# Eclectic-Sheep/sheeprl

Measured on NVIDIA H100. Metric: Dreamer-V3 train-steps/sec (S, bs16 seq64 horizon15, 64x64x3 obs), higher is better.
Workload: dtype f32

## Files before the change

sheeprl_b200/csrc/gemm_tc.cu:

```cuda
#include <cuda.h>
#include <cudaTypedefs.h>

#include <mutex>
#include <unordered_map>

#include "common.cuh"

namespace {

constexpr int BM = 128, BK = 32;
constexpr int NTHREADS = 384;
constexpr int NSPLIT_THREADS = 96;
constexpr int NCONS_WARPS = 8;
constexpr int PRODUCER_REGS = 56, CONSUMER_REGS = 224;
template <int PASSES, bool PRESPLIT> __host__ __device__ constexpr int b_buffers() { return PRESPLIT ? (PASSES == 3 ? 2 : 1) : 3; }
template <int BN, int PASSES, bool PRESPLIT> constexpr int stages_for() {
  return (227 * 1024 - 1024 - 256) / ((BM + b_buffers<PASSES, PRESPLIT>() * BN) * BK * (int)sizeof(float));
}

__device__ __forceinline__ uint32_t smem_u32(const void* p) { return (uint32_t)__cvta_generic_to_shared(p); }

__device__ __forceinline__ void mbar_init(uint64_t* bar, uint32_t count) {
  asm volatile("mbarrier.init.shared::cta.b64 [%0], %1;" ::"r"(smem_u32(bar)), "r"(count) : "memory");
}
__device__ __forceinline__ void mbar_expect_tx(uint64_t* bar, uint32_t bytes) {
  asm volatile("mbarrier.arrive.expect_tx.shared::cta.b64 _, [%0], %1;" ::"r"(smem_u32(bar)), "r"(bytes) : "memory");
}
__device__ __forceinline__ void mbar_arrive(uint64_t* bar) {
  asm volatile("mbarrier.arrive.shared::cta.b64 _, [%0];" ::"r"(smem_u32(bar)) : "memory");
}
__device__ __forceinline__ bool mbar_try_wait(uint64_t* bar, uint32_t parity) {
  uint32_t ok;
  asm volatile(
      "{\n\t"
      ".reg .pred p;\n\t"
      "mbarrier.try_wait.parity.shared::cta.b64 p, [%1], %2;\n\t"
      "selp.u32 %0, 1, 0, p;\n\t"
      "}"
      : "=r"(ok)
      : "r"(smem_u32(bar)), "r"(parity)
      : "memory");
  return ok != 0;
}
__device__ __forceinline__ void mbar_wait(uint64_t* bar, uint32_t parity) {
  if (mbar_try_wait(bar, parity)) return;
  const long long t0 = clock64();
  while (!mbar_try_wait(bar, parity)) {
    if (clock64() - t0 > 2000000000LL) asm volatile("trap;");
  }
}
__device__ __forceinline__ bool elect_one() {
  uint32_t pred;
  asm volatile(
      "{\n\t"
      ".reg .pred p;\n\t"
      "elect.sync _|p, 0xffffffff;\n\t"
      "selp.u32 %0, 1, 0, p;\n\t"
      "}"
      : "=r"(pred));
  return pred != 0;
}
__device__ __forceinline__ void tma_load_2d(void* smem_dst, const CUtensorMap* map, uint64_t* bar, int c0, int c1) {
  asm volatile(
      "cp.async.bulk.tensor.2d.shared::cluster.global.mbarrier::complete_tx::bytes [%0], [%1, {%3, %4}], [%2];" ::"r"(
          smem_u32(smem_dst)),
      "l"(map), "r"(smem_u32(bar)), "r"(c0), "r"(c1)
      : "memory");
}
__device__ __forceinline__ void tma_load_4d(void* smem_dst, const CUtensorMap* map, uint64_t* bar, int c0, int c1, int c2,
                                            int c3) {
  asm volatile(
      "cp.async.bulk.tensor.4d.shared::cluster.global.mbarrier::complete_tx::bytes [%0], [%1, {%3, %4, %5, %6}], [%2];" ::"r"(
          smem_u32(smem_dst)),
      "l"(map), "r"(smem_u32(bar)), "r"(c0), "r"(c1), "r"(c2), "r"(c3)
      : "memory");
}

__device__ __forceinline__ void wgmma_tf32(float (&d)[32], const uint32_t (&a)[4], uint64_t desc_b, int scale_d) {
  asm volatile(
      "{\n\t.reg .pred p;\n\tsetp.ne.b32 p, %37, 0;\n\twgmma.mma_async.sync.aligned.m64n64k8.f32.tf32.tf32 {%0, %1, %2, %3, %4, %5, %6, %7, %8, %9, %10, %11, %12, %13, %14, %15, %16, %17, %18, %19, %20, %21, %22, %23, %24, %25, %26, %27, %28, %29, %30, %31}, {%32, %33, %34, %35}, %36, p, 1, 1;\n\t}"
      : "+f"(d[0]), "+f"(d[1]), "+f"(d[2]), "+f"(d[3]), "+f"(d[4]), "+f"(d[5]), "+f"(d[6]), "+f"(d[7]), "+f"(d[8]), "+f"(d[9]), "+f"(d[10]), "+f"(d[11]), "+f"(d[12]), "+f"(d[13]), "+f"(d[14]), "+f"(d[15]), "+f"(d[16]), "+f"(d[17]), "+f"(d[18]), "+f"(d[19]), "+f"(d[20]), "+f"(d[21]), "+f"(d[22]), "+f"(d[23]), "+f"(d[24]), "+f"(d[25]), "+f"(d[26]), "+f"(d[27]), "+f"(d[28]), "+f"(d[29]), "+f"(d[30]), "+f"(d[31])
      : "r"(a[0]), "r"(a[1]), "r"(a[2]), "r"(a[3]), "l"(desc_b), "r"(scale_d));
}
__device__ __forceinline__ void wgmma_tf32(float (&d)[64], const uint32_t (&a)[4], uint64_t desc_b, int scale_d) {
  asm volatile(
      "{\n\t.reg .pred p;\n\tsetp.ne.b32 p, %69, 0;\n\twgmma.mma_async.sync.aligned.m64n128k8.f32.tf32.tf32 {%0, %1, %2, %3, %4, %5, %6, %7, %8, %9, %10, %11, %12, %13, %14, %15, %16, %17, %18, %19, %20, %21, %22, %23, %24, %25, %26, %27, %28, %29, %30, %31, %32, %33, %34, %35, %36, %37, %38, %39, %40, %41, %42, %43, %44, %45, %46, %47, %48, %49, %50, %51, %52, %53, %54, %55, %56, %57, %58, %59, %60, %61, %62, %63}, {%64, %65, %66, %67}, %68, p, 1, 1;\n\t}"
      : "+f"(d[0]), "+f"(d[1]), "+f"(d[2]), "+f"(d[3]), "+f"(d[4]), "+f"(d[5]), "+f"(d[6]), "+f"(d[7]), "+f"(d[8]), "+f"(d[9]), "+f"(d[10]), "+f"(d[11]), "+f"(d[12]), "+f"(d[13]), "+f"(d[14]), "+f"(d[15]), "+f"(d[16]), "+f"(d[17]), "+f"(d[18]), "+f"(d[19]), "+f"(d[20]), "+f"(d[21]), "+f"(d[22]), "+f"(d[23]), "+f"(d[24]), "+f"(d[25]), "+f"(d[26]), "+f"(d[27]), "+f"(d[28]), "+f"(d[29]), "+f"(d[30]), "+f"(d[31]), "+f"(d[32]), "+f"(d[33]), "+f"(d[34]), "+f"(d[35]), "+f"(d[36]), "+f"(d[37]), "+f"(d[38]), "+f"(d[39]), "+f"(d[40]), "+f"(d[41]), "+f"(d[42]), "+f"(d[43]), "+f"(d[44]), "+f"(d[45]), "+f"(d[46]), "+f"(d[47]), "+f"(d[48]), "+f"(d[49]), "+f"(d[50]), "+f"(d[51]), "+f"(d[52]), "+f"(d[53]), "+f"(d[54]), "+f"(d[55]), "+f"(d[56]), "+f"(d[57]), "+f"(d[58]), "+f"(d[59]), "+f"(d[60]), "+f"(d[61]), "+f"(d[62]), "+f"(d[63])
      : "r"(a[0]), "r"(a[1]), "r"(a[2]), "r"(a[3]), "l"(desc_b), "r"(scale_d));
}
__device__ __forceinline__ void wgmma_fence() { asm volatile("wgmma.fence.sync.aligned;" ::: "memory"); }
__device__ __forceinline__ void wgmma_commit() { asm volatile("wgmma.commit_group.sync.aligned;" ::: "memory"); }
__device__ __forceinline__ void wgmma_wait_all() { asm volatile("wgmma.wait_group.sync.aligned 0;" ::: "memory"); }
template <int N>
__device__ __forceinline__ void fence_regs(float (&r)[N]) {
#pragma unroll
  for (int i = 0; i < N; ++i) asm volatile("" : "+f"(r[i])::"memory");
}
template <int N, int W>
__device__ __forceinline__ void fence_regs(uint32_t (&r)[N][W]) {
#pragma unroll
  for (int i = 0; i < N; ++i)
#pragma unroll
    for (int j = 0; j < W; ++j) asm volatile("" : "+r"(r[i][j])::"memory");
}

__device__ __forceinline__ uint64_t make_desc(uint32_t smem_addr) {
  uint64_t d = 0;
  d |= (uint64_t)((smem_addr & 0x3FFFF) >> 4);
  d |= (uint64_t)1 << 16;
  d |= (uint64_t)(1024 >> 4) << 32;
  d |= (uint64_t)1 << 62;
  return d;
}

__device__ __forceinline__ uint32_t kmajor_off(int r, int k) {
  return (uint32_t)(r * 128 + ((((k >> 2) ^ r) & 7) << 4) + (k & 3) * 4);
}
__device__ __forceinline__ uint32_t mnmajor_off(int r, int k) {
  return (uint32_t)((r >> 5) * 4096 + k * 128 + (((((r & 31) >> 2) ^ k) & 7) << 4) + (r & 3) * 4);
}

template <int BN, int PASSES, bool PRESPLIT>
struct Smem;
template <int BN, int PASSES>
struct Smem<BN, PASSES, false> {
  static constexpr int STAGES = stages_for<BN, PASSES, false>();
  float a[STAGES][BM * BK];
  float b[STAGES][BN * BK];
  float b_hi[STAGES][BN * BK];
  float b_lo[STAGES][BN * BK];
  uint64_t full[STAGES], split[STAGES], empty[STAGES];
};
template <int BN, int PASSES>
struct Smem<BN, PASSES, true> {
  static constexpr int STAGES = stages_for<BN, PASSES, true>();
  float a[STAGES][BM * BK];
  float b_hi[STAGES][BN * BK];
  float b_lo[PASSES == 3 ? STAGES : 1][PASSES == 3 ? BN * BK : 256];
  uint64_t full[STAGES], empty[STAGES];
};

constexpr int CH = 4;

constexpr int MODE_GEMM = 0, MODE_DOWN = 1, MODE_UP = 2;
constexpr int MODE_UP4 = 3;
constexpr int GROUP_M = 16;
struct TileGeo {
  int mode;
  int h, w, NB;
  int bw, bh, bn;
  int tiles_x, tiles_y;
  int chunks;
  int Cout;
  int ksplits;
  float* part;
  int mpad, ldw;
  int force_part;
  int passes;
  int a_mn, b_mn;
  int mtiles;
  int ntiles;
  int wg;
};

template <int BN, int PASSES, bool PRESPLIT>
__global__ void __launch_bounds__(NTHREADS, 1)
gemm_tc_kernel(const __grid_constant__ CUtensorMap mapA, const __grid_constant__ CUtensorMap mapB,
               const __grid_constant__ CUtensorMap mapBlo, float* __restrict__ C, const float* __restrict__ bias, int M,
               int N, int K, int ldc, int accumulate, const TileGeo geo) {
  using S = Smem<BN, PASSES, PRESPLIT>;
  constexpr int STAGES = S::STAGES;
  extern __shared__ __align__(1024) unsigned char smem_raw[];
  S& s = *reinterpret_cast<S*>(smem_raw + ((1024u - (smem_u32(smem_raw) & 1023u)) & 1023u));
  const int warp = threadIdx.x >> 5, lane = threadIdx.x & 31;
  const int mtiles = geo.mtiles * geo.ntiles, tstride = gridDim.y;
  auto tile_mn = [&](int id, int& tm, int& tn) {
    if (geo.ntiles == 1) { tm = id; tn = 0; return; }
    const int per = GROUP_M * geo.ntiles, grp = id / per, first = grp * GROUP_M;
    const int gsz = min(GROUP_M, geo.mtiles - first), r = id - grp * per;
    tn = r / gsz;
    tm = first + (r - tn * gsz);
  };
  int kb_base = 0, nkb = (K + BK - 1) / BK;
  if (geo.mode == MODE_GEMM && geo.ksplits > 1) {
    const int per = (nkb + geo.ksplits - 1) / geo.ksplits;
    kb_base = (int)blockIdx.z * per;
    nkb = min(per, nkb - kb_base);
  }
  const int py = (int)blockIdx.z >> 1, px = (int)blockIdx.z & 1;
  auto tile_origin = [&](int id, int& tx0, int& ty0, int& tn0) {
    tx0 = (id % geo.tiles_x) * geo.bw;
    ty0 = ((id / geo.tiles_x) % geo.tiles_y) * geo.bh;
    tn0 = (id / (geo.tiles_x * geo.tiles_y)) * geo.bn;
  };

  if (threadIdx.x == 0) {
    for (int i = 0; i < STAGES; ++i) {
      mbar_init(&s.full[i], 1);
      if constexpr (!PRESPLIT) mbar_init(&s.split[i], NSPLIT_THREADS / 32);
      mbar_init(&s.empty[i], NCONS_WARPS);
    }
    asm volatile("fence.mbarrier_init.release.cluster;" ::: "memory");
  }
  __syncthreads();

  if (warp < 4) {
    asm volatile("setmaxnreg.dec.sync.aligned.u32 %0;" ::"n"(PRODUCER_REGS));
    if (warp == 0) {
      const bool leader = elect_one();
      constexpr uint32_t STAGE_TX = (uint32_t)((BM + (PRESPLIT ? b_buffers<PASSES, true>() : 1) * BN) * BK * sizeof(float));
      auto load_b_kmajor = [&](int st, int k, int n) {
        if constexpr (PRESPLIT) {
          tma_load_2d(s.b_hi[st], &mapB, &s.full[st], k, n);
          if (PASSES == 3) tma_load_2d(s.b_lo[st], &mapBlo, &s.full[st], k, n);
        } else {
          tma_load_2d(s.b[st], &mapB, &s.full[st], k, n);
        }
      };
      int it = 0;
      for (int tile = blockIdx.y; tile < mtiles; tile += tstride) {
        int tm, tn;
        tile_mn(tile, tm, tn);
        const int m0 = tm * BM, n0 = tn * BN;
        int tx0 = 0, ty0 = 0, tn0 = 0;
        if (geo.mode != MODE_GEMM) tile_origin(tm, tx0, ty0, tn0);
        for (int kb = 0; kb < nkb; ++kb, ++it) {
          const int st = it % STAGES;
          if (it >= STAGES) mbar_wait(&s.empty[st], ((it / STAGES) - 1) & 1);
          if (leader) {
            mbar_expect_tx(&s.full[st], STAGE_TX);
            if (geo.mode == MODE_GEMM) {
              const int k0 = (kb_base + kb) * BK;
              if (geo.wg) {
                const int x0 = k0 % geo.w, y0 = (k0 / geo.w) % geo.h, i0 = k0 / (geo.w * geo.h);
                for (int j = 0; j < BM / 32; ++j) {
                  const int r0 = m0 + 32 * j, tap = r0 / geo.Cout, ch = r0 - tap * geo.Cout;
                  tma_load_4d(s.a[st] + j * 1024, &mapA, &s.full[st], ch, 2 * x0 - 1 + (tap & 3), 2 * y0 - 1 + (tap >> 2), i0);
                }
              } else if (!geo.a_mn) tma_load_2d(s.a[st], &mapA, &s.full[st], k0, m0);
              else
                for (int j = 0; j < BM / 32; ++j) tma_load_2d(s.a[st] + j * 1024, &mapA, &s.full[st], m0 + 32 * j, k0);
              if (PRESPLIT || !geo.b_mn) load_b_kmajor(st, k0, n0);
              else if constexpr (!PRESPLIT)
                for (int j = 0; j < BN / 32; ++j) tma_load_2d(s.b[st] + j * 1024, &mapB, &s.full[st], n0 + 32 * j, k0);
            } else {
              const int tap = kb / geo.chunks, ch = (kb - tap * geo.chunks) * BK;
              int x, y;
              if (geo.mode == MODE_DOWN)     { x = 2 * tx0 - 1 + (tap & 3); y = 2 * ty0 - 1 + (tap >> 2); }
              else if (geo.mode == MODE_UP4) { x = tx0 + (tap % 3) - 1;     y = ty0 + (tap / 3) - 1; }
              else                           { x = tx0 + px - (tap & 1);    y = ty0 + py - (tap >> 1); }
              tma_load_4d(s.a[st], &mapA, &s.full[st], ch, x, y, tn0);
              load_b_kmajor(st, kb * BK, n0 + (geo.mode == MODE_UP ? (int)blockIdx.z * geo.Cout : 0));
            }
          }
          __syncwarp();
        }
      }
    } else if constexpr (!PRESPLIT) {
      const int t = threadIdx.x - 32;
      int ntl = 0;
      for (int tile = blockIdx.y; tile < mtiles; tile += tstride) ++ntl;
      const int total_kb = ntl * nkb;
      const bool b_mn = geo.b_mn != 0;
      for (int kb = 0; kb < total_kb; ++kb) {
        const int st = kb % STAGES;
        mbar_wait(&s.full[st], (kb / STAGES) & 1);
        const char* raw = reinterpret_cast<const char*>(s.b[st]);
        char* bh = reinterpret_cast<char*>(s.b_hi[st]);
        char* bl = reinterpret_cast<char*>(s.b_lo[st]);
#pragma unroll 4
        for (int w = t; w < BN * BK / 4; w += NSPLIT_THREADS) {
          int n, kc;
          float4 v;
          if (!b_mn) {
            n = w >> 3; kc = w & 7;
            v = *reinterpret_cast<const float4*>(raw + kmajor_off(n, 4 * kc));
          } else {
            n = w % BN; kc = w / BN;
            v.x = *reinterpret_cast<const float*>(raw + mnmajor_off(n, 4 * kc));
            v.y = *reinterpret_cast<const float*>(raw + mnmajor_off(n, 4 * kc + 1));
            v.z = *reinterpret_cast<const float*>(raw + mnmajor_off(n, 4 * kc + 2));
            v.w = *reinterpret_cast<const float*>(raw + mnmajor_off(n, 4 * kc + 3));
          }
          float4 h;
          h.x = __uint_as_float(__float_as_uint(v.x) & 0xffffe000u);
          h.y = __uint_as_float(__float_as_uint(v.y) & 0xffffe000u);
          h.z = __uint_as_float(__float_as_uint(v.z) & 0xffffe000u);
          h.w = __uint_as_float(__float_as_uint(v.w) & 0xffffe000u);
          const uint32_t o = kmajor_off(n, 4 * kc);
          *reinterpret_cast<float4*>(bh + o) = h;
          if (PASSES == 3) *reinterpret_cast<float4*>(bl + o) = make_float4(v.x - h.x, v.y - h.y, v.z - h.z, v.w - h.w);
        }
        asm volatile("fence.proxy.async.shared::cta;" ::: "memory");
        __syncwarp();
        if (lane == 0) mbar_arrive(&s.split[st]);
      }
    }
  } else {
    asm volatile("setmaxnreg.inc.sync.aligned.u32 %0;" ::"n"(CONSUMER_REGS));
    constexpr int NACC = BN / 2;
    const int cw = (warp >> 2) - 1, wq = warp & 3, g = lane >> 2, tq = lane & 3;
    const int r0 = cw * 64 + wq * 16 + g;
    const bool a_mn_tile = geo.a_mn != 0;
    const uint64_t dbh_base = make_desc(smem_u32(s.b_hi[0])), dbl_base = make_desc(smem_u32(s.b_lo[0]));
    constexpr uint64_t STAGE_STEP = (uint64_t)(BN * BK * sizeof(float)) >> 4;
    int it = 0;
    for (int tile = blockIdx.y; tile < mtiles; tile += tstride) {
      int tm, tn;
      tile_mn(tile, tm, tn);
      const int m0 = tm * BM, n0 = tn * BN;
      int tx0 = 0, ty0 = 0, tn0 = 0;
      if (geo.mode != MODE_GEMM) tile_origin(tm, tx0, ty0, tn0);
      float acc[NACC], cacc[NACC];
#pragma unroll
      for (int j = 0; j < NACC; ++j) { acc[j] = 0.f; cacc[j] = 0.f; }
      for (int kb = 0; kb < nkb; ++kb, ++it) {
        const int st = it % STAGES;
        const uint32_t ph = (it / STAGES) & 1;
        mbar_wait(&s.full[st], ph);
        if constexpr (!PRESPLIT) mbar_wait(&s.split[st], ph);
        const char* araw = reinterpret_cast<const char*>(s.a[st]);
        uint32_t ahi[4][4], alo[4][4];
#pragma unroll
        for (int ks = 0; ks < 4; ++ks)
#pragma unroll
          for (int e = 0; e < 4; ++e) {
            const int r = r0 + 8 * (e & 1), k = 8 * ks + tq + 4 * (e >> 1);
            const uint32_t x = *reinterpret_cast<const uint32_t*>(araw + (a_mn_tile ? mnmajor_off(r, k) : kmajor_off(r, k)));
            ahi[ks][e] = x & 0xffffe000u;
            if (PASSES == 3) alo[ks][e] = __float_as_uint(__uint_as_float(x) - __uint_as_float(x & 0xffffe000u));
          }
        const bool chunk_start = (kb % CH) == 0;
        const uint64_t dbh0 = dbh_base + (uint64_t)st * STAGE_STEP, dbl0 = dbl_base + (uint64_t)st * STAGE_STEP;
        fence_regs(cacc);
        fence_regs(ahi);
        if (PASSES == 3) fence_regs(alo);
        wgmma_fence();
#pragma unroll
        for (int ks = 0; ks < 4; ++ks) {
          const uint64_t ob = (uint64_t)ks * 2;
          const int keep = !(chunk_start && ks == 0);
          if (PASSES == 3) {
            wgmma_tf32(cacc, ahi[ks], dbl0 + ob, keep);
            wgmma_tf32(cacc, alo[ks], dbh0 + ob, 1);
            wgmma_tf32(cacc, ahi[ks], dbh0 + ob, 1);
          } else {
            wgmma_tf32(cacc, ahi[ks], dbh0 + ob, keep);
          }
        }
        wgmma_commit();
        wgmma_wait_all();
        fence_regs(cacc);
        fence_regs(ahi);
        if (PASSES == 3) fence_regs(alo);
        __syncwarp();
        if (lane == 0) mbar_arrive(&s.empty[st]);
        if ((kb % CH) == CH - 1 || kb == nkb - 1) {
#pragma unroll
          for (int j = 0; j < NACC; ++j) acc[j] += cacc[j];
        }
      }
#pragma unroll
      for (int hh = 0; hh < 2; ++hh) {
        const int r = r0 + 8 * hh;
        const int row = m0 + r;
        bool row_ok = row < M;
        size_t row_off = (size_t)row * ldc;
        int wi = 0, hi = 0, ni = 0;
        if (geo.mode != MODE_GEMM) {
          wi = r % geo.bw; hi = (r / geo.bw) % geo.bh; ni = r / (geo.bw * geo.bh);
          const int n = tn0 + ni, y = ty0 + hi, x = tx0 + wi;
          row_ok = n < geo.NB;
          if (geo.mode == MODE_DOWN) row_off = (((size_t)n * geo.h + y) * geo.w + x) * (size_t)ldc;
          else row_off = (((size_t)n * (2 * geo.h) + (2 * y + py)) * (2 * geo.w) + (2 * x + px)) * (size_t)ldc;
        }
        if (geo.mode == MODE_UP4) {
          if (!row_ok) continue;
          const size_t n = (size_t)(tn0 + ni);
          const int y = ty0 + hi, x = tx0 + wi;
#pragma unroll
          for (int j = 0; j < NACC / 4; ++j) {
            const int c = 8 * j + 2 * tq, p = c >> 5, ch = c & 31;
            float* dst = C + ((n * (2 * geo.h) + (2 * y + (p >> 1))) * (2 * geo.w) + (2 * x + (p & 1))) * (size_t)32 + ch;
            float2 o = make_float2(acc[4 * j + 2 * hh], acc[4 * j + 2 * hh + 1]);
            if (bias) { o.x += bias[ch]; o.y += bias[ch + 1]; }
            *reinterpret_cast<float2*>(dst) = o;
          }
          continue;
        }
        if (geo.mode == MODE_GEMM && (geo.ksplits > 1 || geo.force_part)) {
          float* prow = geo.part + ((size_t)blockIdx.z * geo.mpad + (size_t)row) * geo.ldw + n0;
#pragma unroll
          for (int j = 0; j < NACC / 4; ++j)
            *reinterpret_cast<float2*>(prow + 8 * j + 2 * tq) = make_float2(acc[4 * j + 2 * hh], acc[4 * j + 2 * hh + 1]);
          continue;
        }
        if (!row_ok) continue;
        float* crow = C + row_off;
#pragma unroll
        for (int j = 0; j < NACC / 4; ++j) {
          const int cb = n0 + 8 * j + 2 * tq;
          float v0 = acc[4 * j + 2 * hh], v1 = acc[4 * j + 2 * hh + 1];
          if (cb + 1 < N && ((reinterpret_cast<uintptr_t>(crow + cb) & 7) == 0)) {
            if (bias) { v0 += bias[cb]; v1 += bias[cb + 1]; }
            if (accumulate) { const float2 q = *reinterpret_cast<const float2*>(crow + cb); v0 += q.x; v1 += q.y; }
            *reinterpret_cast<float2*>(crow + cb) = make_float2(v0, v1);
          } else {
            if (cb < N) crow[cb] = v0 + (bias ? bias[cb] : 0.f) + (accumulate ? crow[cb] : 0.f);
            if (cb + 1 < N) crow[cb + 1] = v1 + (bias ? bias[cb + 1] : 0.f) + (accumulate ? crow[cb + 1] : 0.f);
          }
        }
      }
    }
  }
}

struct MapKey {
  const void* ptr; int rows, cols, ld, box_rows;
  bool operator==(const MapKey& o) const { return ptr == o.ptr && rows == o.rows && cols == o.cols && ld == o.ld && box_rows == o.box_rows; }
};
struct MapHash {
  size_t operator()(const MapKey& k) const {
    size_t h = std::hash<const void*>()(k.ptr);
    h ^= std::hash<long long>()(((long long)k.rows << 32) ^ k.cols) + 0x9e3779b97f4a7c15ull + (h << 6) + (h >> 2);
    h ^= std::hash<long long>()(((long long)k.ld << 8) ^ k.box_rows) + 0x9e3779b97f4a7c15ull + (h << 6) + (h >> 2);
    return h;
  }
};
std::unordered_map<MapKey, CUtensorMap, MapHash> g_maps;
std::mutex g_maps_mu;

typedef CUresult (*EncodeTiledFn)(CUtensorMap*, CUtensorMapDataType, cuuint32_t, void*, const cuuint64_t*, const cuuint64_t*,
                                  const cuuint32_t*, const cuuint32_t*, CUtensorMapInterleave, CUtensorMapSwizzle,
                                  CUtensorMapL2promotion, CUtensorMapFloatOOBfill);
EncodeTiledFn encode_tiled() {
  static EncodeTiledFn fn = nullptr;
  if (!fn) {
    void* p = nullptr;
    cudaDriverEntryPointQueryResult q;
    if (cudaGetDriverEntryPoint("cuTensorMapEncodeTiled", &p, cudaEnableDefault, &q) == cudaSuccess &&
        q == cudaDriverEntryPointSuccess)
      fn = reinterpret_cast<EncodeTiledFn>(p);
  }
  return fn;
}

int get_map(const float* ptr, int rows, int cols, int ld, int box_rows, CUtensorMap* out) {
  MapKey key{ptr, rows, cols, ld, box_rows};
  std::lock_guard<std::mutex> lk(g_maps_mu);
  auto it = g_maps.find(key);
  if (it != g_maps.end()) { *out = it->second; return B200RL_OK; }
  CUtensorMap m;
  cuuint64_t dims[2] = {(cuuint64_t)cols, (cuuint64_t)rows};
  cuuint64_t strides[1] = {(cuuint64_t)ld * sizeof(float)};
  cuuint32_t box[2] = {(cuuint32_t)BK, (cuuint32_t)box_rows};
  cuuint32_t estr[2] = {1, 1};
  EncodeTiledFn enc = encode_tiled();
  if (!enc) { b200rl_set_error("cuTensorMapEncodeTiled is not available from this driver"); return B200RL_ERR_CUDA; }
  CUresult r = enc(&m, CU_TENSOR_MAP_DATA_TYPE_FLOAT32, 2, const_cast<float*>(ptr), dims, strides, box,
                                      estr, CU_TENSOR_MAP_INTERLEAVE_NONE,
                                      CU_TENSOR_MAP_SWIZZLE_128B,
                                      CU_TENSOR_MAP_L2_PROMOTION_L2_256B, CU_TENSOR_MAP_FLOAT_OOB_FILL_NONE);
  if (r != CUDA_SUCCESS) {
    b200rl_set_error("cuTensorMapEncodeTiled failed (%d) for [%d x %d] ld %d", (int)r, rows, cols, ld);
    return B200RL_ERR_CUDA;
  }
  if (g_maps.size() > 4096) g_maps.clear();
  g_maps.emplace(key, m);
  *out = m;
  return B200RL_OK;
}

struct Map4Key {
  const void* ptr; int C, W, H, N, bw, bh, bn, es;
  bool operator==(const Map4Key& o) const {
    return ptr == o.ptr && C == o.C && W == o.W && H == o.H && N == o.N && bw == o.bw && bh == o.bh && bn == o.bn && es == o.es;
  }
};
struct Map4Hash {
  size_t operator()(const Map4Key& k) const {
    size_t h = std::hash<const void*>()(k.ptr);
    const long long v[4] = {((long long)k.C << 32) ^ k.W, ((long long)k.H << 32) ^ k.N, ((long long)k.bw << 32) ^ k.bh,
                            ((long long)k.bn << 32) ^ k.es};
    for (long long x : v) h ^= std::hash<long long>()(x) + 0x9e3779b97f4a7c15ull + (h << 6) + (h >> 2);
    return h;
  }
};
std::unordered_map<Map4Key, CUtensorMap, Map4Hash> g_maps4;

int get_map4(const float* ptr, int C, int W, int H, int N, int bw, int bh, int bn, int es, CUtensorMap* out) {
  Map4Key key{ptr, C, W, H, N, bw, bh, bn, es};
  std::lock_guard<std::mutex> lk(g_maps_mu);
  auto it = g_maps4.find(key);
  if (it != g_maps4.end()) { *out = it->second; return B200RL_OK; }
  CUtensorMap m;
  cuuint64_t dims[4] = {(cuuint64_t)C, (cuuint64_t)W, (cuuint64_t)H, (cuuint64_t)N};
  cuuint64_t strides[3] = {(cuuint64_t)C * 4, (cuuint64_t)C * W * 4, (cuuint64_t)C * W * H * 4};
  cuuint32_t box[4] = {(cuuint32_t)BK, (cuuint32_t)((bw - 1) * es + 1), (cuuint32_t)((bh - 1) * es + 1), (cuuint32_t)bn};
  cuuint32_t estr[4] = {1, (cuuint32_t)es, (cuuint32_t)es, 1};
  EncodeTiledFn enc = encode_tiled();
  if (!enc) { b200rl_set_error("cuTensorMapEncodeTiled is not available from this driver"); return B200RL_ERR_CUDA; }
  CUresult r = enc(&m, CU_TENSOR_MAP_DATA_TYPE_FLOAT32, 4, const_cast<float*>(ptr), dims, strides, box,
                                      estr, CU_TENSOR_MAP_INTERLEAVE_NONE,
// ... 10 lines not shown
}

bool conv_tile(int h, int w, int NB, int* bw, int* bh, int* bn) {
  if (w <= 0 || h <= 0 || (w & (w - 1)) || (h & (h - 1))) return false;
  *bw = w < 128 ? w : 128;
  int rest = 128 / *bw;
  *bh = h < rest ? h : rest;
  *bn = rest / *bh;
  return (w % *bw == 0) && (h % *bh == 0) && (*bw * *bh * *bn == 128) && (NB % *bn == 0);
}

static unsigned persistent_grid_y(int tiles, unsigned gz) {
  const long long total = (long long)tiles * gz;
  if (total <= 2LL * kNumSMs) return (unsigned)tiles;
  unsigned gy = kNumSMs / gz;
  if (gy < 1) gy = 1;
  return gy < (unsigned)tiles ? gy : (unsigned)tiles;
}

__device__ __forceinline__ float tf32_hi(float x) { return __uint_as_float(__float_as_uint(x) & 0xffffe000u); }
__device__ __forceinline__ void store_split(float* P, float* L, long long i, float v) {
  if (L) { const float h = tf32_hi(v); P[i] = h; L[i] = v - h; }
  else P[i] = v;
}

__global__ void tf32_split_kernel(const float* __restrict__ X, float* __restrict__ H, float* __restrict__ L, long long n) {
  const long long i = ((long long)blockIdx.x * blockDim.x + threadIdx.x) * 4;
  if (i + 4 <= n && !((reinterpret_cast<uintptr_t>(X) | reinterpret_cast<uintptr_t>(H) | reinterpret_cast<uintptr_t>(L)) & 15)) {
    const float4 v = *reinterpret_cast<const float4*>(X + i);
    const float4 h = make_float4(tf32_hi(v.x), tf32_hi(v.y), tf32_hi(v.z), tf32_hi(v.w));
    *reinterpret_cast<float4*>(H + i) = h;
    *reinterpret_cast<float4*>(L + i) = make_float4(v.x - h.x, v.y - h.y, v.z - h.z, v.w - h.w);
  } else {
    for (long long j = i; j < i + 4 && j < n; ++j) store_split(H, L, j, X[j]);
  }
}

__global__ void tf32_split_t_kernel(const float* __restrict__ W, float* __restrict__ H, float* __restrict__ L, int rows,
                                    int cols, long long ldw, long long ldt) {
  __shared__ float t[32][33];
  const int c0 = blockIdx.x * 32, r0 = blockIdx.y * 32;
  for (int j = threadIdx.y; j < 32; j += blockDim.y) {
    const int r = r0 + j, c = c0 + threadIdx.x;
    t[j][threadIdx.x] = (r < rows && c < cols) ? W[(long long)r * ldw + c] : 0.f;
  }
  __syncthreads();
  for (int j = threadIdx.y; j < 32; j += blockDim.y) {
    const int c = c0 + j, r = r0 + threadIdx.x;
    if (c < cols && r < ldt) store_split(H, L, (long long)c * ldt + r, t[threadIdx.x][j]);
  }
}

__global__ void conv_pack_down_kernel(const float* __restrict__ W, float* __restrict__ P, float* __restrict__ L, int Cs,
                                      int Cb) {
  const long long idx = (long long)blockIdx.x * blockDim.x + threadIdx.x;
  if (idx >= (long long)Cs * Cb * 16) return;
  const int cb = (int)(idx % Cb);
  const int tap = (int)((idx / Cb) % 16);
  const int cs = (int)(idx / ((long long)Cb * 16));
  store_split(P, L, idx, W[((long long)cs * Cb + cb) * 16 + tap]);
}
__global__ void conv_pack_up_kernel(const float* __restrict__ W, float* __restrict__ P, float* __restrict__ L, int Cs,
                                    int Cb) {
  const long long idx = (long long)blockIdx.x * blockDim.x + threadIdx.x;
  if (idx >= (long long)Cs * Cb * 16) return;
  const int cs = (int)(idx % Cs);
  const int t = (int)((idx / Cs) % 4);
  const int cb = (int)((idx / ((long long)Cs * 4)) % Cb);
  const int par = (int)(idx / ((long long)Cs * 4 * Cb));
  const int py = par >> 1, px = par & 1;
  const int ky = (1 - py) + 2 * (t >> 1), kx = (1 - px) + 2 * (t & 1);
  store_split(P, L, idx, W[((long long)cs * Cb + cb) * 16 + ky * 4 + kx]);
}

__global__ void conv_pack_up4_kernel(const float* __restrict__ W, float* __restrict__ P, float* __restrict__ L, int Cs,
                                     int Cb) {
  const long long idx = (long long)blockIdx.x * blockDim.x + threadIdx.x;
  if (idx >= 36LL * Cs * Cb) return;
  const int cs = (int)(idx % Cs);
  const int shift = (int)((idx / Cs) % 9);
  const int cb = (int)((idx / (9LL * Cs)) % Cb);
  const int par = (int)(idx / (9LL * Cs * Cb));
  const int py = par >> 1, px = par & 1, dy = shift / 3 - 1, dx = shift % 3 - 1;
  const int j = py - dy, i = px - dx;
  float v = 0.f;
  if (j >= 0 && j <= 1 && i >= 0 && i <= 1) v = W[((long long)cs * Cb + cb) * 16 + ((1 - py) + 2 * j) * 4 + (1 - px) + 2 * i];
  store_split(P, L, idx, v);
}
static bool conv_up_merged(int Cb) { return Cb == 32; }

int g_passes = 3;

struct SplitWs {
  float* part = nullptr;
  size_t floats = 0;
};
SplitWs g_split[16];
std::mutex g_split_mu;

int split_workspace(size_t need_floats, cudaStream_t st, float** part) {
  int dev = 0;
  RL_CUDA(cudaGetDevice(&dev));
  RL_CHECK_ARG(dev < 16, "split-K workspace: device index out of range");
  std::lock_guard<std::mutex> lk(g_split_mu);
  SplitWs& w = g_split[dev];
  if (need_floats > w.floats) {
    cudaStreamCaptureStatus cs = cudaStreamCaptureStatusNone;
    RL_CUDA(cudaStreamIsCapturing(st, &cs));
    if (cs != cudaStreamCaptureStatusNone) {
      b200rl_set_error("split-K workspace must grow during stream capture: run the step once eagerly first");
      return B200RL_ERR_CUDA;
    }
    RL_CUDA(cudaDeviceSynchronize());
    if (w.part) RL_CUDA(cudaFree(w.part));
    const size_t n = need_floats + need_floats / 2 > (size_t)16 << 20 ? need_floats + need_floats / 2 : (size_t)16 << 20;
    RL_CUDA(cudaMalloc(&w.part, n * sizeof(float)));
    w.floats = n;
  }
  *part = w.part;
  return B200RL_OK;
}

__global__ void __launch_bounds__(256)
splitk_reduce_kernel(const float* __restrict__ part, float* __restrict__ C, const float* __restrict__ bias, int M, int N,
                     int ldc, int ks, int mpad, int ldw, int accumulate) {
  const int n4 = (N + 3) >> 2;
  const long long idx = (long long)blockIdx.x * blockDim.x + threadIdx.x;
  if (idx >= (long long)M * n4) return;
  const int m = (int)(idx / n4), n = (int)(idx - (long long)m * n4) * 4;
  const float* p = part + (size_t)m * ldw + n;
  float4 acc = make_float4(0.f, 0.f, 0.f, 0.f);
#pragma unroll 4
  for (int z = 0; z < ks; ++z) {
    const float4 v = __ldcg(reinterpret_cast<const float4*>(p + (size_t)z * mpad * ldw));
    acc.x += v.x; acc.y += v.y; acc.z += v.z; acc.w += v.w;
  }
  float* c = C + (size_t)m * ldc + n;
  const float o[4] = {acc.x, acc.y, acc.z, acc.w};
  if (n + 4 <= N && ((reinterpret_cast<uintptr_t>(c) & 15) == 0)) {
    float4 r = acc;
    if (bias) { r.x += bias[n]; r.y += bias[n + 1]; r.z += bias[n + 2]; r.w += bias[n + 3]; }
    if (accumulate) { const float4 q = *reinterpret_cast<const float4*>(c); r.x += q.x; r.y += q.y; r.z += q.z; r.w += q.w; }
    *reinterpret_cast<float4*>(c) = r;
  } else {
    for (int j = 0; j < 4 && n + j < N; ++j) {
      float r = o[j];
      if (bias) r += bias[n + j];
      if (accumulate) r += c[j];
      c[j] = r;
    }
  }
}

#define LAUNCH_GEMM_TC(BN_, PASSES_, PRE_, grid_, st_, ...)                                                          \
  do {                                                                                                               \
    static_assert(sizeof(Smem<BN_, PASSES_, PRE_>) + 1024 <= 227 * 1024, "operand stages exceed shared memory");     \
    const size_t smem__ = sizeof(Smem<BN_, PASSES_, PRE_>) + 1024;                                                   \
    RL_CUDA(cudaFuncSetAttribute(gemm_tc_kernel<BN_, PASSES_, PRE_>, cudaFuncAttributeMaxDynamicSharedMemorySize,     \
                                 (int)smem__));                                                                      \
    gemm_tc_kernel<BN_, PASSES_, PRE_><<<grid_, NTHREADS, smem__, st_>>>(__VA_ARGS__);                                \
  } while (0)
#define DISPATCH_GEMM_TC_PRE(BN_val, passes_val, PRE_, grid_, st_, ...)                        \
  do {                                                                                          \
    if ((BN_val) == 64) {                                                                       \
      if ((passes_val) == 3) LAUNCH_GEMM_TC(64, 3, PRE_, grid_, st_, __VA_ARGS__);              \
      else LAUNCH_GEMM_TC(64, 1, PRE_, grid_, st_, __VA_ARGS__);                                \
    } else {                                                                                    \
      if ((passes_val) == 3) LAUNCH_GEMM_TC(128, 3, PRE_, grid_, st_, __VA_ARGS__);             \
      else LAUNCH_GEMM_TC(128, 1, PRE_, grid_, st_, __VA_ARGS__);                               \
    }                                                                                           \
  } while (0)
#define DISPATCH_GEMM_TC(BN_val, passes_val, presplit_, grid_, st_, ma_, mb_, mb2_, ...)                    \
  do {                                                                                                       \
    if (presplit_) DISPATCH_GEMM_TC_PRE(BN_val, passes_val, true, grid_, st_, ma_, mb_, mb2_, __VA_ARGS__);  \
    else DISPATCH_GEMM_TC_PRE(BN_val, passes_val, false, grid_, st_, ma_, mb_, mb_, __VA_ARGS__);           \
  } while (0)

int launch_conv(int mode, const float* img, const float* Wp, const float* Wlo, float* out, const float* bias, int NB, int h,
                int w, int Cin, int Cout, cudaStream_t st) {
  TileGeo g = {};
  g.mode = mode; g.h = h; g.w = w; g.NB = NB; g.chunks = Cin / BK; g.Cout = Cout; g.ksplits = 1;
  g.passes = g_passes;
  RL_CHECK_ARG(conv_tile(h, w, NB, &g.bw, &g.bh, &g.bn), "image grid not tileable by 128 pixels");
  g.tiles_x = w / g.bw; g.tiles_y = h / g.bh;
  if (mode == MODE_UP && conv_up_merged(Cout)) mode = g.mode = MODE_UP4;
  const int taps = mode == MODE_DOWN ? 16 : (mode == MODE_UP4 ? 9 : 4);
  const int K = taps * Cin;
  CUtensorMap ma, mb;
  if (mode == MODE_DOWN) { if (int rc = get_map4(img, Cin, 2 * w, 2 * h, NB, g.bw, g.bh, g.bn, 2, &ma)) return rc; }
  else                   { if (int rc = get_map4(img, Cin, w, h, NB, g.bw, g.bh, g.bn, 1, &ma)) return rc; }
  const int BN = (mode == MODE_UP4) ? 128 : ((Cout <= 64) ? 64 : 128);
  const int brows = (mode == MODE_UP || mode == MODE_UP4) ? 4 * Cout : Cout;
  if (int rc = get_map(Wp, brows, K, K, BN, &mb)) return rc;
  CUtensorMap mb2 = mb;
  if (Wlo && g.passes == 3) { if (int rc = get_map(Wlo, brows, K, K, BN, &mb2)) return rc; }
  const int mtiles = g.tiles_x * g.tiles_y * (NB / g.bn);
  g.mtiles = mtiles;
  g.ntiles = (mode == MODE_UP4) ? 1 : (Cout + BN - 1) / BN;
  dim3 grid(1, 1, mode == MODE_UP ? 4 : 1);
  grid.y = persistent_grid_y(mtiles * g.ntiles, grid.z);
  const int M = NB * h * w;
  DISPATCH_GEMM_TC(BN, g.passes, Wlo != nullptr, grid, st, ma, mb, mb2, out, bias, M, Cout, K, Cout, 0, g);
  RL_CHECK_LAUNCH();
  return B200RL_OK;
}

}

extern "C" int b200rl_set_matmul_precision(int tf32_passes) {
  RL_CHECK_ARG(tf32_passes == 1 || tf32_passes == 3, "tf32_passes must be 3 (fp32-accurate 3xTF32) or 1 (single TF32 pass)");
  g_passes = tf32_passes;
  return B200RL_OK;
}
extern "C" int b200rl_get_matmul_precision(void) { return g_passes; }

extern "C" long long b200rl_conv_pack_floats(int mode_up, int Cs, int Cb) {
  return (mode_up && conv_up_merged(Cb) ? 36LL : 16LL) * Cs * Cb;
}
extern "C" int b200rl_conv_tc_supported(int mode_up, int NB, int h, int w, int Cs, int Cb) {
  int bw, bh, bn;
  if (!conv_tile(h, w, NB, &bw, &bh, &bn)) return 0;
  const int Cin = mode_up ? Cs : Cb, Cout = mode_up ? Cb : Cs;
  if (Cin % BK != 0 || Cout < 16 || Cout % 4 != 0) return 0;
  return 1;
}
namespace {
int conv_pack_impl(const float* W, float* P, float* L, int mode_up, int Cs, int Cb, cudaStream_t st) {
  const long long n = (long long)Cs * Cb * 16;
  if (mode_up && conv_up_merged(Cb)) conv_pack_up4_kernel<<<ceil_div(36LL * Cs * Cb, 256), 256, 0, st>>>(W, P, L, Cs, Cb);
  else if (mode_up) conv_pack_up_kernel<<<ceil_div(n, 256), 256, 0, st>>>(W, P, L, Cs, Cb);
  else conv_pack_down_kernel<<<ceil_div(n, 256), 256, 0, st>>>(W, P, L, Cs, Cb);
  RL_CHECK_LAUNCH();
  return B200RL_OK;
}
}
extern "C" int b200rl_conv_pack(const float* W, float* Wpacked, int mode_up, int Cs, int Cb, cudaStream_t st) {
  RL_CHECK_ARG(W && Wpacked, "null pointer");
  return conv_pack_impl(W, Wpacked, nullptr, mode_up, Cs, Cb, st);
}
extern "C" int b200rl_conv_pack_split(const float* W, float* Whi, float* Wlo, int mode_up, int Cs, int Cb, cudaStream_t st) {
  RL_CHECK_ARG(W && Whi && Wlo, "null pointer");
  return conv_pack_impl(W, Whi, Wlo, mode_up, Cs, Cb, st);
}
extern "C" int b200rl_conv_down_tc(const float* big, const float* Wpacked, float* small_, int NB, int h, int w, int Cs,
                                   int Cb, cudaStream_t st) {
  RL_CHECK_ARG(big && Wpacked && small_, "null pointer");
  RL_CHECK_ARG(b200rl_conv_tc_supported(0, NB, h, w, Cs, Cb), "shape not eligible for the tensor-core conv path");
  return launch_conv(MODE_DOWN, big, Wpacked, nullptr, small_, nullptr, NB, h, w, Cb, Cs, st);
}
extern "C" int b200rl_conv_up_tc(const float* small_, const float* Wpacked, float* big, const float* bias, int NB, int h,
                                 int w, int Cs, int Cb, cudaStream_t st) {
  RL_CHECK_ARG(big && Wpacked && small_, "null pointer");
  RL_CHECK_ARG(b200rl_conv_tc_supported(1, NB, h, w, Cs, Cb), "shape not eligible for the tensor-core conv path");
  return launch_conv(MODE_UP, small_, Wpacked, nullptr, big, bias, NB, h, w, Cs, Cb, st);
}
extern "C" int b200rl_conv_down_tc_presplit(const float* big, const float* Whi, const float* Wlo, float* small_, int NB,
                                            int h, int w, int Cs, int Cb, cudaStream_t st) {
  RL_CHECK_ARG(big && Whi && Wlo && small_, "null pointer");
  RL_CHECK_ARG(b200rl_conv_tc_supported(0, NB, h, w, Cs, Cb), "shape not eligible for the tensor-core conv path");
  return launch_conv(MODE_DOWN, big, Whi, Wlo, small_, nullptr, NB, h, w, Cb, Cs, st);
}
extern "C" int b200rl_conv_up_tc_presplit(const float* small_, const float* Whi, const float* Wlo, float* big,
                                          const float* bias, int NB, int h, int w, int Cs, int Cb, cudaStream_t st) {
  RL_CHECK_ARG(big && Whi && Wlo && small_, "null pointer");
  RL_CHECK_ARG(b200rl_conv_tc_supported(1, NB, h, w, Cs, Cb), "shape not eligible for the tensor-core conv path");
  return launch_conv(MODE_UP, small_, Whi, Wlo, big, bias, NB, h, w, Cs, Cb, st);
}

extern "C" int b200rl_tf32_split(const float* X, float* Xhi, float* Xlo, long long n, cudaStream_t st) {
  RL_CHECK_ARG(X && Xhi && Xlo, "null pointer");
  RL_CHECK_ARG(n >= 0, "negative length");
  if (n == 0) return B200RL_OK;
  tf32_split_kernel<<<ceil_div((n + 3) / 4, 256), 256, 0, st>>>(X, Xhi, Xlo, n);
  RL_CHECK_LAUNCH();
  return B200RL_OK;
}
extern "C" int b200rl_tf32_split_t(const float* W, float* Thi, float* Tlo, int rows, int cols, long long ldw, long long ldt,
                                   cudaStream_t st) {
  RL_CHECK_ARG(W && Thi && Tlo, "null pointer");
  RL_CHECK_ARG(rows > 0 && cols > 0 && ldw >= cols && ldt >= rows, "bad transposed-split geometry");
  dim3 grid(ceil_div(cols, 32), ceil_div(ldt, 32));
  tf32_split_t_kernel<<<grid, dim3(32, 8), 0, st>>>(W, Thi, Tlo, rows, cols, ldw, ldt);
  RL_CHECK_LAUNCH();
  return B200RL_OK;
}

extern "C" int b200rl_gemm_tc_supported(const float* A, const float* B, int M, int N, int K, int lda, int ldb,
                                        int transA, int transB) {
  (void)transA; (void)transB;
  if (M < 32 || N < 48 || K < 32) return 0;
  if ((lda & 3) || (ldb & 3)) return 0;
  if ((reinterpret_cast<uintptr_t>(A) & 15) || (reinterpret_cast<uintptr_t>(B) & 15)) return 0;
  return 1;
}

namespace {
struct FusedTail { float* part; int ks, mpad, ldw; };

int gemm_tc_impl(const float* A, const float* B, const float* Blo, float* C, const float* bias, int M, int N, int K,
                 int lda, int ldb, int ldc, int transA, int transB, int accumulate, cudaStream_t st, FusedTail* fused) {
  RL_CHECK_ARG(A && B && (C || fused), "null pointer");
  RL_CHECK_ARG(b200rl_gemm_tc_supported(A, B, M, N, K, lda, ldb, transA, transB), "shape not eligible for the tensor-core path");
  RL_CHECK_ARG(!Blo || (transB && !(reinterpret_cast<uintptr_t>(Blo) & 15)), "pre-split B must be 16-byte aligned [N][K] planes");
  const int BN = (N <= 64) ? 64 : 128;
  CUtensorMap ma, mb, mb2;
  if (!transA) { if (int rc = get_map(A, M, K, lda, BM, &ma)) return rc; }
  else         { if (int rc = get_map(A, K, M, lda, 32, &ma)) return rc; }
  if (transB)  { if (int rc = get_map(B, N, K, ldb, BN, &mb)) return rc; }
  else         { if (int rc = get_map(B, K, N, ldb, 32, &mb)) return rc; }
  mb2 = mb;
  if (Blo && g_passes == 3) { if (int rc = get_map(Blo, N, K, ldb, BN, &mb2)) return rc; }
  dim3 grid((N + BN - 1) / BN, (M + BM - 1) / BM);
  TileGeo g = {};
  g.mode = MODE_GEMM;
  g.a_mn = transA ? 1 : 0;
  g.b_mn = transB ? 0 : 1;
  g.ksplits = 1;
  g.passes = g_passes;
  const int tiles = grid.x * grid.y, nkb = (K + BK - 1) / BK;
  if (tiles < 2 * kNumSMs && nkb >= 8) {
    int best = 1;
    float best_t = 1e30f;
    const int max_sp = nkb / 4 < 32 ? nkb / 4 : 32;
    for (int sp = 1; sp <= (max_sp < 1 ? 1 : max_sp); ++sp) {
      const int per = (nkb + sp - 1) / sp, real = (nkb + per - 1) / per;
      const int waves = (tiles * real + kNumSMs - 1) / kNumSMs;
      const float t = waves * (per * 0.8f + 4.0f) + (real > 1 ? 3.0f + 0.3f * real : 0.0f);
      if (t < best_t - 1e-3f) { best_t = t; best = real; }
    }
    g.ksplits = best;
  }
  if (g.ksplits > 1 || fused) {
    grid.z = g.ksplits;
    g.mpad = (int)grid.y * BM;
    g.ldw = (int)grid.x * BN;
    if (int rc = split_workspace((size_t)g.ksplits * g.mpad * g.ldw, st, &g.part)) return rc;
    if (fused) { g.force_part = 1; *fused = FusedTail{g.part, g.ksplits, g.mpad, g.ldw}; }
  }
  g.mtiles = (int)grid.y;
  g.ntiles = (int)grid.x;
  grid.x = 1;
  grid.y = persistent_grid_y(g.mtiles * g.ntiles, grid.z);
  DISPATCH_GEMM_TC(BN, g.passes, Blo != nullptr, grid, st, ma, mb, mb2, C, bias, M, N, K, ldc, accumulate, g);
  RL_CHECK_LAUNCH();
  if (g.ksplits > 1 && !fused) {
    splitk_reduce_kernel<<<ceil_div((long long)M * ((N + 3) / 4), 256), 256, 0, st>>>(g.part, C, bias, M, N, ldc, g.ksplits, g.mpad,
                                                                                      g.ldw, accumulate);
    RL_CHECK_LAUNCH();
  }
  return B200RL_OK;
}

template <int NV>
__global__ void __launch_bounds__(256)
splitk_ln_kernel(const float* __restrict__ part, int ks, int mpad, int ldw, int M, int N, const float* __restrict__ gamma,
// ... 200 lines not shown
```

Measured before the change: 62.13.

## Skip structurally-zero parity blocks in merged UP4 transposed-conv GEMM

For the merged 3x3-shift transposed convolution (UP4) with pre-split 3xTF32 weights, the kernel now loads and multiplies only the 32-column output-parity slices that each shift tap actually contributes to. It uses n32 wgmma instructions per parity slice instead of one n128 instruction over the whole packed weight tile, and sizes TMA boxes and expected transaction bytes per k-block. This cuts both weight traffic and tensor-core work, since the zero blocks in the packed weight matrix are no longer touched. In exchange it issues more, smaller MMA instructions, adds a runtime switch over compile-time parity masks, and zeroes the accumulator explicitly at each chunk start.

```diff
diff --git a/sheeprl_b200/csrc/gemm_tc.cu b/sheeprl_b200/csrc/gemm_tc.cu
--- a/sheeprl_b200/csrc/gemm_tc.cu
+++ b/sheeprl_b200/csrc/gemm_tc.cu
@@ -87,6 +87,12 @@
       "{\n\t.reg .pred p;\n\tsetp.ne.b32 p, %69, 0;\n\twgmma.mma_async.sync.aligned.m64n128k8.f32.tf32.tf32 {%0, %1, %2, %3, %4, %5, %6, %7, %8, %9, %10, %11, %12, %13, %14, %15, %16, %17, %18, %19, %20, %21, %22, %23, %24, %25, %26, %27, %28, %29, %30, %31, %32, %33, %34, %35, %36, %37, %38, %39, %40, %41, %42, %43, %44, %45, %46, %47, %48, %49, %50, %51, %52, %53, %54, %55, %56, %57, %58, %59, %60, %61, %62, %63}, {%64, %65, %66, %67}, %68, p, 1, 1;\n\t}"
       : "+f"(d[0]), "+f"(d[1]), "+f"(d[2]), "+f"(d[3]), "+f"(d[4]), "+f"(d[5]), "+f"(d[6]), "+f"(d[7]), "+f"(d[8]), "+f"(d[9]), "+f"(d[10]), "+f"(d[11]), "+f"(d[12]), "+f"(d[13]), "+f"(d[14]), "+f"(d[15]), "+f"(d[16]), "+f"(d[17]), "+f"(d[18]), "+f"(d[19]), "+f"(d[20]), "+f"(d[21]), "+f"(d[22]), "+f"(d[23]), "+f"(d[24]), "+f"(d[25]), "+f"(d[26]), "+f"(d[27]), "+f"(d[28]), "+f"(d[29]), "+f"(d[30]), "+f"(d[31]), "+f"(d[32]), "+f"(d[33]), "+f"(d[34]), "+f"(d[35]), "+f"(d[36]), "+f"(d[37]), "+f"(d[38]), "+f"(d[39]), "+f"(d[40]), "+f"(d[41]), "+f"(d[42]), "+f"(d[43]), "+f"(d[44]), "+f"(d[45]), "+f"(d[46]), "+f"(d[47]), "+f"(d[48]), "+f"(d[49]), "+f"(d[50]), "+f"(d[51]), "+f"(d[52]), "+f"(d[53]), "+f"(d[54]), "+f"(d[55]), "+f"(d[56]), "+f"(d[57]), "+f"(d[58]), "+f"(d[59]), "+f"(d[60]), "+f"(d[61]), "+f"(d[62]), "+f"(d[63])
       : "r"(a[0]), "r"(a[1]), "r"(a[2]), "r"(a[3]), "l"(desc_b), "r"(scale_d));
+}
+__device__ __forceinline__ void wgmma_tf32_n32(float* d, const uint32_t (&a)[4], uint64_t desc_b) {
+  asm volatile(
+      "wgmma.mma_async.sync.aligned.m64n32k8.f32.tf32.tf32 {%0, %1, %2, %3, %4, %5, %6, %7, %8, %9, %10, %11, %12, %13, %14, %15}, {%16, %17, %18, %19}, %20, 1, 1, 1;"
+      : "+f"(d[0]), "+f"(d[1]), "+f"(d[2]), "+f"(d[3]), "+f"(d[4]), "+f"(d[5]), "+f"(d[6]), "+f"(d[7]), "+f"(d[8]), "+f"(d[9]), "+f"(d[10]), "+f"(d[11]), "+f"(d[12]), "+f"(d[13]), "+f"(d[14]), "+f"(d[15])
+      : "r"(a[0]), "r"(a[1]), "r"(a[2]), "r"(a[3]), "l"(desc_b));
 }
 __device__ __forceinline__ void wgmma_fence() { asm volatile("wgmma.fence.sync.aligned;" ::: "memory"); }
 __device__ __forceinline__ void wgmma_commit() { asm volatile("wgmma.commit_group.sync.aligned;" ::: "memory"); }
@@ -144,6 +150,14 @@
 
 constexpr int MODE_GEMM = 0, MODE_DOWN = 1, MODE_UP = 2;
 constexpr int MODE_UP4 = 3;
+__host__ __device__ constexpr uint32_t up4_parities(int shift) {
+  const uint32_t ys = shift / 3 == 0 ? 1u : (shift / 3 == 1 ? 3u : 2u), xs = shift % 3 == 0 ? 1u : (shift % 3 == 1 ? 3u : 2u);
+  return ((ys & 1u) ? xs : 0u) | ((ys & 2u) ? xs << 2 : 0u);
+}
+static_assert(up4_parities(0) == 1 && up4_parities(1) == 3 && up4_parities(2) == 2 && up4_parities(3) == 5 &&
+                  up4_parities(4) == 15 && up4_parities(5) == 10 && up4_parities(6) == 4 && up4_parities(7) == 12 &&
+                  up4_parities(8) == 8,
+              "UP4 shift -> parity table");
 constexpr int GROUP_M = 16;
 struct TileGeo {
   int mode;
@@ -163,11 +177,30 @@
   int wg;
 };
 
-template <int BN, int PASSES, bool PRESPLIT>
+template <uint32_t PAR>
+__device__ __forceinline__ void up4_kblock(float (&cacc)[64], const uint32_t (&ahi)[4][4], const uint32_t (&alo)[4][4],
+                                           uint64_t dbh0, uint64_t dbl0) {
+  constexpr uint64_t PARITY_STEP = (uint64_t)(32 * BK * sizeof(float)) >> 4;
+  wgmma_fence();
+#pragma unroll
+  for (int ks = 0; ks < 4; ++ks)
+#pragma unroll
+    for (int p = 0; p < 4; ++p) {
+      if (!((PAR >> p) & 1u)) continue;
+      const uint64_t o = (uint64_t)ks * 2 + (uint64_t)p * PARITY_STEP;
+      wgmma_tf32_n32(cacc + 16 * p, ahi[ks], dbl0 + o);
+      wgmma_tf32_n32(cacc + 16 * p, alo[ks], dbh0 + o);
+      wgmma_tf32_n32(cacc + 16 * p, ahi[ks], dbh0 + o);
+    }
+  wgmma_commit();
+}
+
+template <int BN, int PASSES, bool PRESPLIT, bool UP4_SKIP = false>
 __global__ void __launch_bounds__(NTHREADS, 1)
 gemm_tc_kernel(const __grid_constant__ CUtensorMap mapA, const __grid_constant__ CUtensorMap mapB,
                const __grid_constant__ CUtensorMap mapBlo, float* __restrict__ C, const float* __restrict__ bias, int M,
                int N, int K, int ldc, int accumulate, const TileGeo geo) {
+  static_assert(!UP4_SKIP || (BN == 128 && PASSES == 3 && PRESPLIT), "the UP4 skip walk is a 3xTF32 pre-split 128-column tile");
   using S = Smem<BN, PASSES, PRESPLIT>;
   constexpr int STAGES = S::STAGES;
   extern __shared__ __align__(1024) unsigned char smem_raw[];
@@ -228,7 +261,10 @@
           const int st = it % STAGES;
           if (it >= STAGES) mbar_wait(&s.empty[st], ((it / STAGES) - 1) & 1);
           if (leader) {
-            mbar_expect_tx(&s.full[st], STAGE_TX);
+            const uint32_t up4_par = UP4_SKIP ? up4_parities(kb / geo.chunks) : 0u;
+            mbar_expect_tx(&s.full[st], UP4_SKIP ? (uint32_t)((BM + __popc(up4_par) * 32 * b_buffers<PASSES, true>()) * BK *
+                                                              sizeof(float))
+                                                 : STAGE_TX);
             if (geo.mode == MODE_GEMM) {
               const int k0 = (kb_base + kb) * BK;
               if (geo.wg) {
@@ -250,7 +286,15 @@
               else if (geo.mode == MODE_UP4) { x = tx0 + (tap % 3) - 1;     y = ty0 + (tap / 3) - 1; }
               else                           { x = tx0 + px - (tap & 1);    y = ty0 + py - (tap >> 1); }
               tma_load_4d(s.a[st], &mapA, &s.full[st], ch, x, y, tn0);
-              load_b_kmajor(st, kb * BK, n0 + (geo.mode == MODE_UP ? (int)blockIdx.z * geo.Cout : 0));
+              if constexpr (UP4_SKIP) {
+                for (int p = 0; p < 4; ++p)
+                  if ((up4_par >> p) & 1u) {
+                    tma_load_2d(s.b_hi[st] + p * 32 * BK, &mapB, &s.full[st], kb * BK, 32 * p);
+                    tma_load_2d(s.b_lo[st] + p * 32 * BK, &mapBlo, &s.full[st], kb * BK, 32 * p);
+                  }
+              } else {
+                load_b_kmajor(st, kb * BK, n0 + (geo.mode == MODE_UP ? (int)blockIdx.z * geo.Cout : 0));
+              }
             }
           }
           __syncwarp();
@@ -335,20 +379,38 @@
         fence_regs(cacc);
         fence_regs(ahi);
         if (PASSES == 3) fence_regs(alo);
-        wgmma_fence();
-#pragma unroll
-        for (int ks = 0; ks < 4; ++ks) {
-          const uint64_t ob = (uint64_t)ks * 2;
-          const int keep = !(chunk_start && ks == 0);
-          if (PASSES == 3) {
-            wgmma_tf32(cacc, ahi[ks], dbl0 + ob, keep);
-            wgmma_tf32(cacc, alo[ks], dbh0 + ob, 1);
-            wgmma_tf32(cacc, ahi[ks], dbh0 + ob, 1);
-          } else {
-            wgmma_tf32(cacc, ahi[ks], dbh0 + ob, keep);
+        if constexpr (UP4_SKIP) {
+          if (chunk_start) {
+#pragma unroll
+            for (int j = 0; j < NACC; ++j) cacc[j] = 0.f;
           }
+          switch (kb / geo.chunks) {
+            case 0: up4_kblock<up4_parities(0)>(cacc, ahi, alo, dbh0, dbl0); break;
+            case 1: up4_kblock<up4_parities(1)>(cacc, ahi, alo, dbh0, dbl0); break;
+            case 2: up4_kblock<up4_parities(2)>(cacc, ahi, alo, dbh0, dbl0); break;
+            case 3: up4_kblock<up4_parities(3)>(cacc, ahi, alo, dbh0, dbl0); break;
+            case 4: up4_kblock<up4_parities(4)>(cacc, ahi, alo, dbh0, dbl0); break;
+            case 5: up4_kblock<up4_parities(5)>(cacc, ahi, alo, dbh0, dbl0); break;
+            case 6: up4_kblock<up4_parities(6)>(cacc, ahi, alo, dbh0, dbl0); break;
+            case 7: up4_kblock<up4_parities(7)>(cacc, ahi, alo, dbh0, dbl0); break;
+            default: up4_kblock<up4_parities(8)>(cacc, ahi, alo, dbh0, dbl0); break;
+          }
+        } else {
+          wgmma_fence();
+#pragma unroll
+          for (int ks = 0; ks < 4; ++ks) {
+            const uint64_t ob = (uint64_t)ks * 2;
+            const int keep = !(chunk_start && ks == 0);
+            if (PASSES == 3) {
+              wgmma_tf32(cacc, ahi[ks], dbl0 + ob, keep);
+              wgmma_tf32(cacc, alo[ks], dbh0 + ob, 1);
+              wgmma_tf32(cacc, ahi[ks], dbh0 + ob, 1);
+            } else {
+              wgmma_tf32(cacc, ahi[ks], dbh0 + ob, keep);
+            }
+          }
+          wgmma_commit();
         }
-        wgmma_commit();
         wgmma_wait_all();
         fence_regs(cacc);
         fence_regs(ahi);
@@ -665,14 +727,15 @@
   }
 }
 
-#define LAUNCH_GEMM_TC(BN_, PASSES_, PRE_, grid_, st_, ...)                                                          \
+#define LAUNCH_GEMM_TC_K(BN_, PASSES_, PRE_, UP4_, grid_, st_, ...)                                                 \
   do {                                                                                                               \
     static_assert(sizeof(Smem<BN_, PASSES_, PRE_>) + 1024 <= 227 * 1024, "operand stages exceed shared memory");     \
     const size_t smem__ = sizeof(Smem<BN_, PASSES_, PRE_>) + 1024;                                                   \
-    RL_CUDA(cudaFuncSetAttribute(gemm_tc_kernel<BN_, PASSES_, PRE_>, cudaFuncAttributeMaxDynamicSharedMemorySize,     \
+    RL_CUDA(cudaFuncSetAttribute(gemm_tc_kernel<BN_, PASSES_, PRE_, UP4_>, cudaFuncAttributeMaxDynamicSharedMemorySize, \
                                  (int)smem__));                                                                      \
-    gemm_tc_kernel<BN_, PASSES_, PRE_><<<grid_, NTHREADS, smem__, st_>>>(__VA_ARGS__);                                \
+    gemm_tc_kernel<BN_, PASSES_, PRE_, UP4_><<<grid_, NTHREADS, smem__, st_>>>(__VA_ARGS__);                          \
   } while (0)
+#define LAUNCH_GEMM_TC(BN_, PASSES_, PRE_, grid_, st_, ...) LAUNCH_GEMM_TC_K(BN_, PASSES_, PRE_, false, grid_, st_, __VA_ARGS__)
 #define DISPATCH_GEMM_TC_PRE(BN_val, passes_val, PRE_, grid_, st_, ...)                        \
   do {                                                                                          \
     if ((BN_val) == 64) {                                                                       \
@@ -704,16 +767,22 @@
   else                   { if (int rc = get_map4(img, Cin, w, h, NB, g.bw, g.bh, g.bn, 1, &ma)) return rc; }
   const int BN = (mode == MODE_UP4) ? 128 : ((Cout <= 64) ? 64 : 128);
   const int brows = (mode == MODE_UP || mode == MODE_UP4) ? 4 * Cout : Cout;
-  if (int rc = get_map(Wp, brows, K, K, BN, &mb)) return rc;
+  const bool skip = mode == MODE_UP4 && Wlo && g.passes == 3;
+  const int bbox = skip ? 32 : BN;
+  if (int rc = get_map(Wp, brows, K, K, bbox, &mb)) return rc;
   CUtensorMap mb2 = mb;
-  if (Wlo && g.passes == 3) { if (int rc = get_map(Wlo, brows, K, K, BN, &mb2)) return rc; }
+  if (Wlo && g.passes == 3) { if (int rc = get_map(Wlo, brows, K, K, bbox, &mb2)) return rc; }
   const int mtiles = g.tiles_x * g.tiles_y * (NB / g.bn);
   g.mtiles = mtiles;
   g.ntiles = (mode == MODE_UP4) ? 1 : (Cout + BN - 1) / BN;
   dim3 grid(1, 1, mode == MODE_UP ? 4 : 1);
   grid.y = persistent_grid_y(mtiles * g.ntiles, grid.z);
   const int M = NB * h * w;
-  DISPATCH_GEMM_TC(BN, g.passes, Wlo != nullptr, grid, st, ma, mb, mb2, out, bias, M, Cout, K, Cout, 0, g);
+  if (skip) {
+    LAUNCH_GEMM_TC_K(128, 3, true, true, grid, st, ma, mb, mb2, out, bias, M, Cout, K, Cout, 0, g);
+  } else {
+    DISPATCH_GEMM_TC(BN, g.passes, Wlo != nullptr, grid, st, ma, mb, mb2, out, bias, M, Cout, K, Cout, 0, g);
+  }
   RL_CHECK_LAUNCH();
   return B200RL_OK;
 }
```

Result: no change. 62.25 (median of 6 runs) (+0.2%).
